# ouguangjun/Leg-KILO

Measured on NVIDIA H100. Metric: LiDAR point-iterations/sec through the ESKF point-to-plane update, higher is better.
Workload: dtype f64

## Files before the change

leg-kilo_b200/csrc/lk_fused.cu:

```cuda
#include "lk_insert.cuh"
#include "lk_kernels.h"
#include "lk_obs.cuh"
#include "lk_pass.cuh"
#include "lk_predict.cuh"
#include "lk_solve.cuh"

namespace lk {

namespace {

#define FT(slot) do { if (a.trace && threadIdx.x == 0 && (slot) < 32) a.trace[(size_t)blockIdx.x * 32 + (slot)] = gtime(); } while (0)
#define FTI(slot) do { if (it_global < 3) FT(slot); } while (0)
#define FTS(slot) do { if (a.trace && blockIdx.x == 0 && threadIdx.x == 0 && k < 64) a.trace[(size_t)gridDim.x * 32 + (size_t)k * 8 + (slot)] = gtime(); } while (0)
#ifndef LK_HOP_TRACE
#define LK_HOP_TRACE 0
#endif
#define FT_HOPS() ((LK_HOP_TRACE && a.trace && it_global < 3) \
                       ? a.trace + (size_t)gridDim.x * 32 + 64 * 8 + (size_t)blockIdx.x * 16 + it_global * LL_HOP_SLOTS : nullptr)

constexpr int BLOCK = FB;
constexpr int WARPS = BLOCK / 32;

struct PredictScratch {
    double F[900];
    double T[900];
    double Ps[900];
    ObsScratch obs;
};

template <bool HOT>
struct FusedSmemT {
    BlockFilter f;
    ScanConst sc;
    double slice[WARPS * 32];
    double clk[2];
    union {
        PredictScratch pr;
        PassSmem<BLOCK, HOT> pass;
    } u;
};
typedef FusedSmemT<true> FusedSmem;

struct FusedSmemIns {
    FusedSmemT<false> base;
    WarpTile wt[WARPS];
    MapDev md;
    Globals g;
};

__device__ __noinline__ void fused_insert_phase2(FusedSmemIns* si, const uint32_t* touched, const int* iroot, const DevPoint* ipts,
                                                 int* pend, uint32_t n_touched, uint32_t n_bucket) {
    const int lane = threadIdx.x & 31, warp = threadIdx.x >> 5;
    MapDev md = si->md;
    WarpTile* wt = si->wt + warp;
    for (uint32_t t = blockIdx.x * (uint32_t)WARPS + (uint32_t)warp; t < n_touched; t += gridDim.x * (uint32_t)WARPS)
        warp_insert_root_scan(md, si->g, wt, __ldcg(&touched[t]), iroot, ipts, n_bucket, pend, lane);
}

static_assert(sizeof(PredictScratch) <= sizeof(((PassSmem<BLOCK, true>*)0)->tile) &&
                  sizeof(PredictScratch) <= sizeof(((PassSmem<BLOCK, false>*)0)->tile),
              "predict scratch must not reach the mbarriers");
static_assert(sizeof(FusedSmemIns) <= 227 * 1024, "one block per SM");
static_assert(sizeof(FusedSmem) + 1024 <= 132 * 1024, "the batch-of-one kernel's stack frames must fit in L1");

int carveout_percent(size_t smem, int dev) {
    int per_sm = 0, per_block = 0;
    cudaDeviceGetAttribute(&per_sm, cudaDevAttrMaxSharedMemoryPerMultiprocessor, dev);
    cudaDeviceGetAttribute(&per_block, cudaDevAttrReservedSharedMemoryPerBlock, dev);
    if (per_sm <= 0) return 100;
    const size_t need = smem + (size_t)per_block;
    const int pct = (int)((need * 100 + (size_t)per_sm - 1) / (size_t)per_sm);
    return pct < 100 ? pct : 100;
}

template <class SM>
__device__ __noinline__ void fused_predict(SM* sm, const double* Q, double dtc, double dt) {
    if (dtc != 0.0) {
        build_F(sm->u.pr.F, sm->f.x, dtc);
        cov_predict(sm->f.P, sm->u.pr.F, sm->u.pr.T, sm->u.pr.Ps, Q, dtc);
    }
    if (dt != 0.0) {
        if (threadIdx.x == 0) state_predict(sm->f.x, dt);
    }
    fence_proxy_async();
    __syncthreads();
}

template <class SM>
__device__ __noinline__ void fused_drain_queue(SM* sm, const FusedArgs& a, uint32_t& mi, double t_bucket) {
    bool drained = false;
    while (mi < a.n_meas) {
        const double ts = a.imu ? a.imu[mi].stamp : a.kin[mi].stamp;
        if (!(ts < t_bucket)) break;
        block_predict_to(&sm->f, sm->clk, ts, sm->u.pr.F, sm->u.pr.T, sm->u.pr.Ps, a.Q);
        if (a.imu) block_obs_imu<BLOCK>(&sm->f, &sm->u.pr.obs, a.imu + mi, &a.ecfg, a.gravity, a.acc_norm);
        else block_obs_kinimu<BLOCK>(&sm->f, &sm->u.pr.obs, a.kin + mi, &a.ecfg, a.gravity, a.acc_norm);
        if (threadIdx.x == 0) sm->clk[1] = ts;
        __syncthreads();
        ++mi;
        drained = true;
    }
    if (drained) {
        fence_proxy_async();
        __syncthreads();
    }
}

__device__ __forceinline__ float4 world_out(const double* X, double pix, double piy, double piz, bool updated) {
    float4 o;
    o.x = (float)(X[0] * pix + X[1] * piy + X[2] * piz + X[9]);
    o.y = (float)(X[3] * pix + X[4] * piy + X[5] * piz + X[10]);
    o.z = (float)(X[6] * pix + X[7] * piy + X[8] * piz + X[11]);
    o.w = updated ? 255.0f : 0.0f;
    return o;
}

template <class SM>
__device__ __forceinline__ void store_state(SM* sm, const FusedArgs& a, uint32_t n_eff) {
    const int tid = threadIdx.x;
    if (tid < 36) a.x[(size_t)a.scan * 36 + tid] = sm->f.x[tid];
    if (tid < 2) reinterpret_cast<double*>(a.clk + a.scan)[tid] = sm->clk[tid];
    if (tid == 0) {
        a.n_eff[a.scan] = n_eff;
        *a.status = (*reinterpret_cast<volatile uint32_t*>(a.ll.stall) ? 1u : 0u) | (*reinterpret_cast<volatile uint32_t*>(&lk_stall_note[0]) ? 2u : 0u);
    }
}

template <class SM>
__device__ __noinline__ void fused_finish(SM* sm, const FusedArgs& a, const StepInit& in, uint32_t n_chunks, uint32_t it_global,
                                          bool updated, bool dep_waited) {
    const int tid = threadIdx.x;
    const uint32_t fi = blockIdx.x - n_chunks, nf = gridDim.x - n_chunks;
    if (!dep_waited) asm volatile("griddepcontrol.wait;" ::: "memory");
    ll_sum_chunk_rows<WARPS>(a.ll, it_global & 1u, a.epoch + it_global, n_chunks, sm->u.pr.F, sm->f.acc);
    FTI(3 + it_global * 4);
    const uint32_t n = block_solve_state(&sm->f);
    FTI(4 + it_global * 4);
    if (n > 0) {
        updated = true;
        if (tid == 0) sm->clk[1] = in.t_bucket;
    }
    const float4* pts = a.pts;
    if (a.pts_copy) {
        __threadfence();
        pts = a.pts_copy;
    }
    constexpr int U = 8;
    const uint32_t step = nf * BLOCK;
    for (uint32_t i0 = in.pt_begin + fi * BLOCK + tid; i0 < in.pt_end; i0 += U * step) {
        float4 q[U];
#pragma unroll
        for (int u = 0; u < U; ++u)
            if (i0 + u * step < in.pt_end) q[u] = __ldcg(pts + i0 + u * step);
#pragma unroll
        for (int u = 0; u < U; ++u)
            if (i0 + u * step < in.pt_end) {
                PointCtx p;
                imu_point(q[u], a.g, p);
                a.world[i0 + u * step] = world_out(sm->f.x, p.pix, p.piy, p.piz, updated);
            }
    }
    FT(20);
    if (n > 0) cov_prep(&sm->f, BLOCK);
    __syncthreads();
    for (uint32_t e = fi * BLOCK + tid; e < 900; e += nf * BLOCK)
        a.P[(size_t)a.scan * 900 + e] = n > 0 ? cov_entry(&sm->f, (int)e) : sm->f.P[e];
    FT(21);
    if (fi == 0) store_state(sm, a, n);
    FT(22);
}

template <bool INL> struct InlineSel { typedef FusedInline type; };
template <> struct InlineSel<false> { typedef FusedNoInline type; };

__device__ __forceinline__ void grid_sync(const FusedArgs& a, uint32_t& sync_idx) {
    __threadfence();
    __syncthreads();
    if (threadIdx.x < 32) (void)ll_allreduce(a.ll, sync_idx & 1u, a.epoch + sync_idx, blockIdx.x, gridDim.x, 0.0, (int)threadIdx.x);
    ++sync_idx;
    __syncthreads();
    __threadfence();
    fence_proxy_async_global();
}

template <bool OBS, bool INL, bool INS>
__global__ void __launch_bounds__(BLOCK, 1) k_scan_fused(const __grid_constant__ FusedArgs a,
                                                         const __grid_constant__ typename InlineSel<INL>::type inl) {
    extern __shared__ __align__(16) unsigned char smem_raw[];
    FusedSmemT<!INS>* sm = reinterpret_cast<FusedSmemT<!INS>*>(smem_raw);
    const int tid = threadIdx.x, lane = tid & 31, warp = tid >> 5;
    const uint32_t scan = a.scan;
    const bool finisher = blockIdx.x + a.finishers >= gridDim.x;
    asm volatile("griddepcontrol.launch_dependents;" ::: "memory");
    FT(0);
    {
        const double* Pin;
        const double* xin;
        const double* cin;
        if constexpr (INL) { Pin = inl.P; xin = inl.x; cin = inl.clk; }
        else { Pin = a.P_in + (size_t)scan * 900; xin = a.x_in + (size_t)scan * 36; cin = reinterpret_cast<const double*>(a.clk_in + scan); }
        if (a.slim_p && !finisher && (a.finishers || blockIdx.x != 0)) {
            if (tid < 180) sm->f.P[(tid / 6) * 30 + tid % 6] = Pin[(tid / 6) * 30 + tid % 6];
        } else {
            for (int e = tid; e < 900; e += BLOCK) sm->f.P[e] = Pin[e];
        }
        if (tid < 36) sm->f.x[tid] = xin[tid];
        if (tid < 2) sm->clk[tid] = cin[tid];
    }
    if constexpr (INS) {
        FusedSmemIns* si = reinterpret_cast<FusedSmemIns*>(smem_raw);
        WarpTile* wt = si->wt + warp;
        if (lane == 0) {
            mbar_init(&wt->bar, 1);
            wt->phase = 0;
        }
        if (tid == 0) si->md = a.md;
        if (tid < (int)(sizeof(Globals) / 4)) reinterpret_cast<uint32_t*>(&si->g)[tid] = reinterpret_cast<const uint32_t*>(&a.g)[tid];
    }
    pass_init(&sm->u.pass);
    FT(1);
    uint32_t n_eff_total = 0;
    uint32_t phase = 0;
    uint32_t it_global = 0;
    uint32_t cslot = 0;
    uint32_t mi = 0;
    bool dep_waited = false;

    for (uint32_t k = 0; k < a.n_steps; ++k) {
        StepInit in;
        if constexpr (INL) in = inl.steps[k];
        else in = a.inits[(size_t)k * a.batch + scan];
        if (!in.active) continue;
        const uint32_t n_chunks = in.chunk_end - in.chunk_begin;
        const uint32_t my_start = in.pt_begin + blockIdx.x * (uint32_t)BLOCK;
        const uint32_t my_count = blockIdx.x < n_chunks ? min((uint32_t)BLOCK, in.pt_end - my_start) : 0u;
        float4 pre = make_float4(0.f, 0.f, 0.f, 0.f);
        if ((uint32_t)tid < my_count) pre = __ldg(a.pts + my_start + tid);
        FTS(0);
        if constexpr (OBS) fused_drain_queue(sm, a, mi, in.t_bucket);
        FTS(1);
        const double dtc = in.t_bucket - sm->clk[1];
        const double dt = in.t_bucket - sm->clk[0];
        if (dtc != 0.0 || dt != 0.0) fused_predict(sm, a.Q, dtc, dt);
        if (tid == 0) sm->clk[0] = in.t_bucket;
        FTS(2);
        bool updated = false, cov_pending = false;
        uint32_t n_last = 0;
        LaneCache lc;
        lc.have = 0;
        const bool more_steps = k + 1 < a.n_steps;
        for (int it = 0; it < a.iters; ++it, ++it_global) {
            scan_const_from(&sm->f, &sm->sc);
            __syncthreads();
            double acc[32];
#pragma unroll
            for (int i = 0; i < 32; ++i) acc[i] = 0.0;
            if (!a.lane_cache && lc.have == 2) lc.have = 1;
            points_pass<BLOCK, INS>(&sm->u.pass, phase, my_count, sm->sc, a.mv, a.g, lc, pre,
                                    [&](uint32_t, const Row& row) { accumulate_row(row, acc); });
            FTI(14 + it_global);
            const double tot = warp_transpose_sum(acc, lane);
            sm->slice[warp * 32 + lane] = tot;
            __syncthreads();
            FTI(2 + it_global * 4);
            if (it == 0) FTS(3);
            const bool last = it == a.iters - 1;
            if (!OBS && !INS && a.finishers && last) {
                if (finisher) {
                    fused_finish(sm, a, in, n_chunks, it_global, updated, dep_waited);
                } else {
                    if (!dep_waited) asm volatile("griddepcontrol.wait;" ::: "memory");
                    if (a.pts_copy) {
                        if ((uint32_t)tid < my_count) a.pts_copy[my_start + tid] = pre;
                        __threadfence();
                        __syncthreads();
                    }
                    if (warp == 0) {
                        double v = 0.0;
#pragma unroll
                        for (int w = 0; w < WARPS; ++w) v += sm->slice[w * 32 + lane];
                        ll_publish_row(a.ll, it_global & 1u, a.epoch + it_global, blockIdx.x, v, lane);
                    }
                }
                FT(31);
                return;
            }
            if (warp == 0) {
                double v = 0.0;
#pragma unroll
                for (int w = 0; w < WARPS; ++w) v += sm->slice[w * 32 + lane];
                if (!dep_waited) {
                    FT(23);
                    asm volatile("griddepcontrol.wait;" ::: "memory");
                    FT(24);
                }
                sm->f.acc[lane] = ll_allreduce(a.ll, it_global & 1u, a.epoch + it_global, blockIdx.x, n_chunks, v, lane, FT_HOPS(),
                                               a.finishers, it_global >= 2);
            }
            dep_waited = true;
            __syncthreads();
            FTI(3 + it_global * 4);
            if (it == 0) FTS(4);
            const uint32_t n = block_solve_state(&sm->f);
            FTI(4 + it_global * 4);
            if (n > 0) {
                updated = true;
                if (tid == 0) sm->clk[1] = in.t_bucket;
                if (last) cov_pending = INS || more_steps || blockIdx.x == 0;
            }
            n_last = n;
        }
        n_eff_total += n_last;
        FTS(5);
        if constexpr (!INS) {
            if ((uint32_t)tid < my_count) a.world[my_start + tid] = world_out(sm->f.x, lc.pix, lc.piy, lc.piz, updated);
            FT(20);
            if (cov_pending) block_cov_update<BLOCK>(&sm->f);
        } else {
            if (cov_pending) block_cov_update<BLOCK>(&sm->f);
            __syncthreads();
            scan_const_from(&sm->f, &sm->sc);
            __syncthreads();
            MapDev md = a.md;
            const uint32_t n_bucket = in.pt_end - in.pt_begin;
            if ((uint32_t)tid < my_count) {
                DevPoint p;
                make_insert_point(lc.pix, lc.piy, lc.piz, lc.pbx, lc.pby, lc.pbz, sm->sc, a.g, p);
                const uint32_t li = my_start + tid - in.pt_begin;
                a.ipts[li] = p;
                float4 o;
                o.x = (float)p.pw[0]; o.y = (float)p.pw[1]; o.z = (float)p.pw[2];
                o.w = updated ? 255.0f : 0.0f;
                a.world[my_start + tid] = o;
                a.iroot[li] = insert_register_point(md, a.g, p, a.pend, a.touched, &a.ins_counters[cslot]);
            }
            grid_sync(a, it_global);
            FTS(6);
            {
                const uint32_t n_touched = __ldcg(&a.ins_counters[cslot]);
                if (blockIdx.x == 0 && tid == 0) a.ins_counters[cslot ^ 1u] = 0;
                fused_insert_phase2(reinterpret_cast<FusedSmemIns*>(smem_raw), a.touched, a.iroot, a.ipts, a.pend, n_touched, n_bucket);
                cslot ^= 1u;
            }
            grid_sync(a, it_global);
            FTS(7);
        }
    }
    FT(30);
    if (blockIdx.x == 0) {
        if (!dep_waited) asm volatile("griddepcontrol.wait;" ::: "memory");
        __syncthreads();
        for (int e = tid; e < 900; e += BLOCK) a.P[(size_t)scan * 900 + e] = sm->f.P[e];
        store_state(sm, a, n_eff_total);
    }
    FT(31);
}

template <bool OBS, bool INL, bool INS>
cudaError_t launch_one(const FusedArgs& a, const FusedInline* inl, uint32_t grid, cudaStream_t s, int mode) {
    auto kern = k_scan_fused<OBS, INL, INS>;
    constexpr size_t SMEM = INS ? sizeof(FusedSmemIns) : sizeof(FusedSmem);
    static PerDeviceOnce once;
    if (once.first()) {
        int dev = 0;
        cudaGetDevice(&dev);
        cudaError_t e = cudaFuncSetAttribute(kern, cudaFuncAttributeMaxDynamicSharedMemorySize, (int)SMEM);
        if (e != cudaSuccess) return e;
        e = cudaFuncSetAttribute(kern, cudaFuncAttributePreferredSharedMemoryCarveout, carveout_percent(SMEM, dev));
        if (e != cudaSuccess) return e;
    }
    typename InlineSel<INL>::type local_inl;
    const typename InlineSel<INL>::type* ip;
    if constexpr (INL) ip = inl;
    else { local_inl.unused = 0; ip = &local_inl; }
    if (mode == FUSED_LAUNCH_COOPERATIVE) {
        void* params[] = {(void*)&a, (void*)ip};
        return cudaLaunchCooperativeKernel((const void*)kern, dim3(grid), dim3(BLOCK), params, SMEM, s);
    }
    cudaLaunchConfig_t cfg = {};
    cfg.gridDim = dim3(grid);
    cfg.blockDim = dim3(BLOCK);
    cfg.dynamicSmemBytes = SMEM;
    cfg.stream = s;
    cudaLaunchAttribute at[1];
    at[0].id = cudaLaunchAttributeProgrammaticStreamSerialization;
    at[0].val.programmaticStreamSerializationAllowed = 1;
    cfg.attrs = at;
    cfg.numAttrs = mode == FUSED_LAUNCH_PDL ? 1 : 0;
    return cudaLaunchKernelEx(&cfg, kern, a, *ip);
}

}

size_t fused_smem_bytes() { return sizeof(FusedSmem); }

int fused_read_stall(uint32_t out[8]) {
    if (cudaMemcpyFromSymbol(out, lk_stall_note, 32) != cudaSuccess) return -1;
    if (out[0]) {
        const uint32_t z[8] = {0, 0, 0, 0, 0, 0, 0, 0};
        cudaMemcpyToSymbol(lk_stall_note, z, 32);
    }
    return 0;
}

int fused_max_blocks(int device) {
    static int cached[64];
    static bool have[64];
    if (device >= 0 && device < 64 && have[device]) return cached[device];
    int sms = 0;
    cudaDeviceGetAttribute(&sms, cudaDevAttrMultiProcessorCount, device);
    int n = sms < LL_MAX_CHUNKS ? sms : LL_MAX_CHUNKS;
    if (device >= 0 && device < 64) { cached[device] = n; have[device] = true; }
    return n;
}

cudaError_t launch_scan_fused(const FusedArgs& a, const FusedInline* inl, uint32_t grid, cudaStream_t s, int mode) {
    const bool obs = a.n_meas > 0;
    if (a.insert) {
        if (inl) return cudaErrorInvalidValue;
        return obs ? launch_one<true, false, true>(a, inl, grid, s, mode) : launch_one<false, false, true>(a, inl, grid, s, mode);
    }
    if (obs) return inl ? launch_one<true, true, false>(a, inl, grid, s, mode) : launch_one<true, false, false>(a, inl, grid, s, mode);
    return inl ? launch_one<false, true, false>(a, inl, grid, s, mode) : launch_one<false, false, false>(a, inl, grid, s, mode);
}

}
```

leg-kilo_b200/csrc/lk_llsync.cuh:

```cuda
#pragma once
#include <cuda_runtime.h>
#include <stdint.h>

#include "lk_async.cuh"

namespace lk {

constexpr int LK_GROUP = 8;
constexpr int LL_ROW = 32;
constexpr int LL_MAX_CHUNKS = 160;
constexpr int LL_MAX_GROUPS = (LL_MAX_CHUNKS + LK_GROUP - 1) / LK_GROUP;
constexpr int LL_REPLICAS = 4;
constexpr int LL_COPIES = LL_REPLICAS + 1;
constexpr int LL_MAX_FINISHERS = 24;

struct LLView {
    ulonglong2* chunk_rows;
    ulonglong2* group_rows;
    uint32_t* stall;
    uint32_t* acks;
};
constexpr size_t LL_ROWS_BYTES = (size_t)2 * (LL_MAX_CHUNKS + LL_COPIES * LL_MAX_GROUPS) * LL_ROW * sizeof(ulonglong2);
constexpr size_t LL_BYTES = LL_ROWS_BYTES + 64 + 2 * LL_MAX_FINISHERS * sizeof(uint32_t);
constexpr uint32_t LL_SPIN_LIMIT = 1u << 23;
constexpr int LL_HOP_SLOTS = 5;

__device__ __forceinline__ void ll_store(ulonglong2* p, double v, uint32_t tag) {
    const unsigned long long b = (unsigned long long)__double_as_longlong(v);
    const unsigned long long t = (unsigned long long)tag << 32;
    const unsigned long long w0 = (b & 0xffffffffull) | t, w1 = (b >> 32) | t;
    asm volatile("st.relaxed.gpu.global.v2.u64 [%0], {%1, %2};" ::"l"(p), "l"(w0), "l"(w1) : "memory");
}

__device__ __forceinline__ void ll_give_up(uint32_t* stall, uint32_t tag, uint32_t r0, uint32_t n, int lane) {
    if (atomicCAS(stall, 0u, 1u) == 0u) {
        stall[1] = blockIdx.x; stall[2] = tag; stall[3] = r0; stall[4] = n; stall[5] = (uint32_t)lane;
        __threadfence();
    }
}

template <int N, bool KEEP>
__device__ __forceinline__ double ll_sum_rows(const ulonglong2* rows, uint32_t r0, uint32_t n, uint32_t tag, int lane,
                                              uint32_t* stall, uint32_t& rounds, double first = 0.0, bool have_first = false) {
    static_assert(N <= 32, "one bit per row");
    const ulonglong2* p = rows + (size_t)r0 * LL_ROW + lane;
    unsigned long long w0[N], w1[N];
    const unsigned long long want = ((unsigned long long)tag << 32);
    uint32_t spins = 0;
    if constexpr (!KEEP) {
        bool all;
        do {
#pragma unroll
            for (int k = 0; k < N; ++k)
                if ((uint32_t)k < n && !(have_first && k == 0))
                    asm volatile("ld.relaxed.gpu.global.v2.u64 {%0, %1}, [%2];" : "=l"(w0[k]), "=l"(w1[k]) : "l"(p + (size_t)k * LL_ROW));
            all = true;
#pragma unroll
            for (int k = 0; k < N; ++k)
                if ((uint32_t)k < n && !(have_first && k == 0))
                    all = all && ((w0[k] & 0xffffffff00000000ull) == want) && ((w1[k] & 0xffffffff00000000ull) == want);
            ++spins;
            if (!all && ((spins & 0xfffu) == 0u)) {
                if (spins >= LL_SPIN_LIMIT || *reinterpret_cast<volatile uint32_t*>(stall) != 0u) {
                    ll_give_up(stall, tag, r0, n, lane);
                    break;
                }
            }
        } while (!all);
    } else {
        uint32_t todo = (n >= 32u ? 0xffffffffu : (1u << n) - 1u) & (have_first ? ~1u : ~0u);
        while (true) {
#pragma unroll
            for (int k = 0; k < N; ++k)
                if ((todo >> k) & 1u)
                    asm volatile("ld.relaxed.gpu.global.v2.u64 {%0, %1}, [%2];" : "=l"(w0[k]), "=l"(w1[k]) : "l"(p + (size_t)k * LL_ROW));
#pragma unroll
            for (int k = 0; k < N; ++k)
                if (((todo >> k) & 1u) && ((w0[k] & 0xffffffff00000000ull) == want) && ((w1[k] & 0xffffffff00000000ull) == want))
                    todo &= ~(1u << k);
            ++spins;
            if (todo == 0u) break;
            if ((spins & 0xfffu) == 0u) {
                if (spins >= LL_SPIN_LIMIT || *reinterpret_cast<volatile uint32_t*>(stall) != 0u) {
                    ll_give_up(stall, tag, r0, n, lane);
                    break;
                }
            }
        }
    }
    rounds = spins;
    double s = 0.0;
#pragma unroll
    for (int k = 0; k < N; ++k)
        if ((uint32_t)k < n) {
            const double v = (have_first && k == 0) ? first : __longlong_as_double((long long)((w0[k] & 0xffffffffull) | (w1[k] << 32)));
            s += v;
        }
    return s;
}

__device__ __forceinline__ void ll_wait_acks(const uint32_t* acks, uint32_t fin, uint32_t tag, int lane, uint32_t* stall) {
    uint32_t spins = 0;
    bool mine = (uint32_t)lane >= fin;
    while (!__all_sync(0xffffffffu, mine)) {
        if (!mine) {
            uint32_t w;
            asm volatile("ld.acquire.gpu.global.u32 %0, [%1];" : "=r"(w) : "l"(acks + lane) : "memory");
            mine = w == tag;
        }
        if ((++spins & 0xfffu) == 0u && (spins >= LL_SPIN_LIMIT || *reinterpret_cast<volatile uint32_t*>(stall) != 0u)) {
            ll_give_up(stall, tag, 0, fin, lane);
            break;
        }
    }
}

__device__ __forceinline__ double ll_allreduce(const LLView& ll, uint32_t parity, uint32_t tag, uint32_t b, uint32_t n_chunks,
                                               double v, int lane, unsigned long long* hops = nullptr, uint32_t fin = 0,
                                               bool acks_due = false) {
    constexpr size_t COPY = (size_t)LL_MAX_GROUPS * LL_ROW;
    ulonglong2* crows = ll.chunk_rows + (size_t)parity * LL_MAX_CHUNKS * LL_ROW;
    ulonglong2* grows = ll.group_rows + (size_t)parity * LL_COPIES * COPY;
    uint32_t* acks = ll.acks + (size_t)parity * LL_MAX_FINISHERS;
    const uint32_t n_groups = (n_chunks + LK_GROUP - 1) / LK_GROUP;
    uint32_t r1 = 0, r2 = 0;
    if (b < n_chunks) {
        if ((b % LK_GROUP) == 0) {
            if (hops && lane == 0) hops[0] = gtime();
            const uint32_t n = min((uint32_t)LK_GROUP, n_chunks - b);
            const double s = ll_sum_rows<LK_GROUP, false>(crows, b, n, tag, lane, ll.stall, r1, v, true);
            if (hops && lane == 0) hops[1] = gtime();
            ulonglong2* g = grows + (size_t)(b / LK_GROUP) * LL_ROW + lane;
            if (fin && acks_due) ll_wait_acks(acks, fin, tag - 2u, lane, ll.stall);
#pragma unroll
            for (int r = 0; r < LL_REPLICAS; ++r) ll_store(g + (size_t)r * COPY, s, tag);
            if (fin) ll_store(g + (size_t)LL_REPLICAS * COPY, s, tag);
            if (hops && lane == 0) hops[2] = gtime();
        } else {
            ll_store(crows + (size_t)b * LL_ROW + lane, v, tag);
            if (hops && lane == 0) hops[0] = gtime();
        }
    }
    const bool finisher = fin && b >= n_chunks;
    const double t = ll_sum_rows<LL_MAX_GROUPS, true>(grows + (size_t)(finisher ? LL_REPLICAS : b % LL_REPLICAS) * COPY, 0, n_groups,
                                                      tag, lane, ll.stall, r2);
    if (finisher) {
        __syncwarp();
        if (lane == 0) asm volatile("st.release.gpu.global.u32 [%0], %1;" ::"l"(acks + (b - n_chunks)), "r"(tag) : "memory");
    }
    if (hops) {
        r1 = __reduce_max_sync(0xffffffffu, r1);
        r2 = __reduce_max_sync(0xffffffffu, r2);
        if (lane == 0) {
            hops[3] = gtime();
            hops[4] = (unsigned long long)r1 | ((unsigned long long)r2 << 32);
        }
    }
    return t;
}

__device__ __forceinline__ void ll_publish_row(const LLView& ll, uint32_t parity, uint32_t tag, uint32_t b, double v, int lane) {
    ll_store(ll.chunk_rows + ((size_t)parity * LL_MAX_CHUNKS + b) * LL_ROW + lane, v, tag);
}

template <int NWARPS>
__device__ __forceinline__ void ll_sum_chunk_rows(const LLView& ll, uint32_t parity, uint32_t tag, uint32_t n_chunks, double* gs,
                                                  double* out) {
    const int tid = threadIdx.x, lane = tid & 31, warp = tid >> 5;
    const ulonglong2* crows = ll.chunk_rows + (size_t)parity * LL_MAX_CHUNKS * LL_ROW;
    const uint32_t n_groups = (n_chunks + LK_GROUP - 1) / LK_GROUP;
    for (uint32_t g = (uint32_t)warp; g < n_groups; g += NWARPS) {
        uint32_t rounds;
        gs[g * 32 + lane] = ll_sum_rows<LK_GROUP, false>(crows, g * LK_GROUP, min((uint32_t)LK_GROUP, n_chunks - g * LK_GROUP), tag,
                                                         lane, ll.stall, rounds);
    }
    __syncthreads();
    if (tid < 32) {
        double t = 0.0;
        for (uint32_t g = 0; g < n_groups; ++g) t += gs[g * 32 + tid];
        out[tid] = t;
    }
    __syncthreads();
}

}
```

Before: 3.124 billion.

## Prefetch finisher points into shared memory before waiting on chunk sums

Finisher blocks now load and IMU-transform their first batch of points into a shared-memory staging area, reusing the tile region, before they spin on the chunk-row reduction. Once the state solve finishes, those staged points are written out directly, so point loading overlaps the cross-block wait. Separately, each warp in the chunk-row sum now polls two groups at once with the bitmask polling variant, which halves the serial waits per warp. The cost is more shared-memory aliasing, which static asserts guard, and more registers for the 16-row poll.

Measured after the change: 3.301 billion (median of 6 runs). +5.7%, better.

```diff
diff --git a/leg-kilo_b200/csrc/lk_fused.cu b/leg-kilo_b200/csrc/lk_fused.cu
--- a/leg-kilo_b200/csrc/lk_fused.cu
+++ b/leg-kilo_b200/csrc/lk_fused.cu
@@ -126,12 +126,44 @@
     }
 }
 
+typedef PassSmem<BLOCK, true> PassHot;
+typedef PassSmem<BLOCK, false> PassNodes;
+constexpr size_t FIN_GS_BYTES = (size_t)LL_MAX_GROUPS * 32 * sizeof(double);
+constexpr uint32_t FIN_STAGE = (uint32_t)((sizeof(PassHot::tile) - FIN_GS_BYTES) / (3 * sizeof(double)));
+static_assert(offsetof(PredictScratch, F) == 0 && offsetof(PassHot, tile) == 0 && offsetof(PassNodes, tile) == 0,
+              "the group sums and the staging area start at the tiles");
+static_assert(FIN_GS_BYTES + 3 * sizeof(double) * FIN_STAGE <= sizeof(PassHot::tile) &&
+                  sizeof(PassHot::tile) <= sizeof(PassNodes::tile) && sizeof(PassHot::tile) <= offsetof(PassHot, bar),
+              "the finishers' staging area must stay inside the tiles, clear of the mbarriers");
+
 template <class SM>
 __device__ __noinline__ void fused_finish(SM* sm, const FusedArgs& a, const StepInit& in, uint32_t n_chunks, uint32_t it_global,
                                           bool updated, bool dep_waited) {
     const int tid = threadIdx.x;
     const uint32_t fi = blockIdx.x - n_chunks, nf = gridDim.x - n_chunks;
     if (!dep_waited) asm volatile("griddepcontrol.wait;" ::: "memory");
+    constexpr int U = 8;
+    const uint32_t step = nf * BLOCK;
+    const uint32_t first = in.pt_begin + fi * BLOCK + tid;
+    double* st = reinterpret_cast<double*>(reinterpret_cast<unsigned char*>(&sm->u) + FIN_GS_BYTES);
+    const uint32_t n_pts = first < in.pt_end ? (in.pt_end - first + step - 1) / step : 0u;
+    const uint32_t n_st = a.pts_copy ? 0u : min(n_pts, (FIN_STAGE - (uint32_t)tid + BLOCK - 1) / BLOCK);
+    for (uint32_t j0 = 0; j0 < n_st; j0 += U) {
+        float4 q[U];
+#pragma unroll
+        for (int u = 0; u < U; ++u)
+            if (j0 + u < n_st) q[u] = __ldcg(a.pts + first + (j0 + u) * step);
+#pragma unroll
+        for (int u = 0; u < U; ++u)
+            if (j0 + u < n_st) {
+                PointCtx p;
+                imu_point(q[u], a.g, p);
+                const uint32_t l = (j0 + u) * BLOCK + tid;
+                st[l] = p.pix;
+                st[FIN_STAGE + l] = p.piy;
+                st[2 * FIN_STAGE + l] = p.piz;
+            }
+    }
     ll_sum_chunk_rows<WARPS>(a.ll, it_global & 1u, a.epoch + it_global, n_chunks, sm->u.pr.F, sm->f.acc);
     FTI(3 + it_global * 4);
     const uint32_t n = block_solve_state(&sm->f);
@@ -140,14 +172,16 @@
         updated = true;
         if (tid == 0) sm->clk[1] = in.t_bucket;
     }
+    for (uint32_t j = 0; j < n_st; ++j) {
+        const uint32_t l = j * BLOCK + tid;
+        a.world[first + j * step] = world_out(sm->f.x, st[l], st[FIN_STAGE + l], st[2 * FIN_STAGE + l], updated);
+    }
     const float4* pts = a.pts;
     if (a.pts_copy) {
         __threadfence();
         pts = a.pts_copy;
     }
-    constexpr int U = 8;
-    const uint32_t step = nf * BLOCK;
-    for (uint32_t i0 = in.pt_begin + fi * BLOCK + tid; i0 < in.pt_end; i0 += U * step) {
+    for (uint32_t i0 = first + n_st * step; i0 < in.pt_end; i0 += U * step) {
         float4 q[U];
 #pragma unroll
         for (int u = 0; u < U; ++u)
diff --git a/leg-kilo_b200/csrc/lk_llsync.cuh b/leg-kilo_b200/csrc/lk_llsync.cuh
--- a/leg-kilo_b200/csrc/lk_llsync.cuh
+++ b/leg-kilo_b200/csrc/lk_llsync.cuh
@@ -39,9 +39,10 @@
     }
 }
 
-template <int N, bool KEEP>
+template <int N, bool KEEP, int SPLIT = N>
 __device__ __forceinline__ double ll_sum_rows(const ulonglong2* rows, uint32_t r0, uint32_t n, uint32_t tag, int lane,
-                                              uint32_t* stall, uint32_t& rounds, double first = 0.0, bool have_first = false) {
+                                              uint32_t* stall, uint32_t& rounds, double first = 0.0, bool have_first = false,
+                                              double* hi = nullptr) {
     static_assert(N <= 32, "one bit per row");
     const ulonglong2* p = rows + (size_t)r0 * LL_ROW + lane;
     unsigned long long w0[N], w1[N];
@@ -91,11 +92,18 @@
     rounds = spins;
     double s = 0.0;
 #pragma unroll
-    for (int k = 0; k < N; ++k)
+    for (int k = 0; k < SPLIT; ++k)
         if ((uint32_t)k < n) {
             const double v = (have_first && k == 0) ? first : __longlong_as_double((long long)((w0[k] & 0xffffffffull) | (w1[k] << 32)));
             s += v;
         }
+    if constexpr (SPLIT < N) {
+        double s2 = 0.0;
+#pragma unroll
+        for (int k = SPLIT; k < N; ++k)
+            if ((uint32_t)k < n) s2 += __longlong_as_double((long long)((w0[k] & 0xffffffffull) | (w1[k] << 32)));
+        *hi = s2;
+    }
     return s;
 }
 
@@ -169,10 +177,12 @@
     const int tid = threadIdx.x, lane = tid & 31, warp = tid >> 5;
     const ulonglong2* crows = ll.chunk_rows + (size_t)parity * LL_MAX_CHUNKS * LL_ROW;
     const uint32_t n_groups = (n_chunks + LK_GROUP - 1) / LK_GROUP;
-    for (uint32_t g = (uint32_t)warp; g < n_groups; g += NWARPS) {
+    for (uint32_t g = 2u * (uint32_t)warp; g < n_groups; g += 2u * NWARPS) {
         uint32_t rounds;
-        gs[g * 32 + lane] = ll_sum_rows<LK_GROUP, false>(crows, g * LK_GROUP, min((uint32_t)LK_GROUP, n_chunks - g * LK_GROUP), tag,
-                                                         lane, ll.stall, rounds);
+        double hi;
+        gs[g * 32 + lane] = ll_sum_rows<2 * LK_GROUP, true, LK_GROUP>(crows, g * LK_GROUP, min(2u * LK_GROUP, n_chunks - g * LK_GROUP),
+                                                                       tag, lane, ll.stall, rounds, 0.0, false, &hi);
+        if (g + 1 < n_groups) gs[(g + 1) * 32 + lane] = hi;
     }
     __syncthreads();
     if (tid < 32) {
```
